# tenpy/cyten

Measured on AMD Instinct MI355X. Metric: block-sparse tdot+SVD GFLOP/s (fp64), higher is better.
Workload: dtype f64

## Files before the change

### cyten_amd/csrc/blocked_qr.hip

```cpp
#include "blocked_qr.h"
#include "qr_strip_chunks.h"

#include <algorithm>
#include <cstdlib>
#include <utility>

namespace cyb {
namespace {

#define GLOBAL_AS __attribute__((address_space(1)))
typedef GLOBAL_AS double* gp;
typedef const GLOBAL_AS double* gcp;
typedef double d4 __attribute__((ext_vector_type(4)));

constexpr int PNT = 512;
constexpr int PNW = PNT / 64;

__device__ __forceinline__ double wave_sum(double v)
{
#pragma unroll
    for (int o = 32; o > 0; o >>= 1) v += __shfl_xor(v, o);
    return v;
}

// ... 81 lines not shown
            else if (i > col) val = (tj != 0.0) ? x[i - col] * scale : 0.0;
            v[i] = val;
        }
        __syncthreads();
        if (tj != 0.0) {
            for (int c = col + 1 + wave; c < j0 + pw; c += PNW) {
                gp a = Ac + (int64_t)c * ld + col;
                gcp vv = v + col;
                double dot = 0.0;
                for (int i = lane; i < L; i += 64) dot += vv[i] * a[i];
                dot = wave_sum(dot) * tj;
                for (int i = lane; i < L; i += 64) a[i] -= dot * vv[i];
            }
        }
        for (int i = wave; i < jj; i += PNW) {
            gcp vi = V + (int64_t)(j0 + i) * ld;
            double dot = 0.0;
            for (int r = col + lane; r < m; r += 64) dot += vi[r] * v[r];
            dot = wave_sum(dot);
            if (lane == 0) z[i] = dot;
        }
        __syncthreads();
        if (tid < jj) {
            double acc = 0.0;
            for (int l = tid; l < jj; ++l) acc += Ts[tid][l] * z[l];
            Ts[tid][jj] = -tj * acc;
        }
        if (tid == 0) Ts[jj][jj] = tj;
        __syncthreads();
    }
    for (int e = tid; e < NBK * NBK; e += PNT) ((gp)d.T)[e] = Ts[e / NBK][e % NBK];
}

#ifndef CYB_QR_READLANE
#define CYB_QR_READLANE 1
#endif
constexpr int RP_NT = 512;
constexpr int RP_RPT = 3;
constexpr int RP_NW = RP_NT / 64;

__device__ __forceinline__ double dshfl_xor(double v, int m) { return __shfl_xor(v, m); }

#ifndef CYB_QR_REDUCE_DPP
#define CYB_QR_REDUCE_DPP 1
#endif
#if CYB_QR_REDUCE_DPP
__device__ __forceinline__ void dswap32(double& a, double& b)
{
    const auto lo = __builtin_amdgcn_permlane32_swap((unsigned)__double2loint(a), (unsigned)__double2loint(b), false, false);
    const auto hi = __builtin_amdgcn_permlane32_swap((unsigned)__double2hiint(a), (unsigned)__double2hiint(b), false, false);
    a = __hiloint2double((int)hi[0], (int)lo[0]);
    b = __hiloint2double((int)hi[1], (int)lo[1]);
}
__device__ __forceinline__ void dswap16(double& a, double& b)
{
    const auto lo = __builtin_amdgcn_permlane16_swap((unsigned)__double2loint(a), (unsigned)__double2loint(b), false, false);
    const auto hi = __builtin_amdgcn_permlane16_swap((unsigned)__double2hiint(a), (unsigned)__double2hiint(b), false, false);
    a = __hiloint2double((int)hi[0], (int)lo[0]);
    b = __hiloint2double((int)hi[1], (int)lo[1]);
}
template <int CTRL, int BANKS>
__device__ __forceinline__ double ddpp(double old, double src)
{
    const int lo = __builtin_amdgcn_update_dpp(__double2loint(old), __double2loint(src), CTRL, 0xf, BANKS, false);
    const int hi = __builtin_amdgcn_update_dpp(__double2hiint(old), __double2hiint(src), CTRL, 0xf, BANKS, false);
    return __hiloint2double(hi, lo);
}
__device__ __forceinline__ double reduce_scatter16(double (&v)[16], int )
{
    double a[8];
#pragma unroll
    for (int i = 0; i < 8; ++i) {
        double x = v[i], y = v[i + 8];
        dswap32(x, y);
        a[i] = x + y;
    }
    double b[4];
#pragma unroll
    for (int i = 0; i < 4; ++i) {
        double x = a[i], y = a[i + 4];
        dswap16(x, y);
        b[i] = x + y;
    }
    constexpr int ROW_MIRROR = 0x140, ROW_HALF_MIRROR = 0x141;
    double c[2];
#pragma unroll
    for (int i = 0; i < 2; ++i) {
        const double p = ddpp<ROW_MIRROR, 0xc>(b[i], b[i + 2]);
        const double q = ddpp<ROW_MIRROR, 0x3>(b[i + 2], b[i]);
        c[i] = p + q;
    }
    const double p = ddpp<ROW_HALF_MIRROR, 0xa>(c[0], c[1]);
    const double q = ddpp<ROW_HALF_MIRROR, 0x5>(c[1], c[0]);
    double d = p + q;
    d += ddpp<0x4e, 0xf>(d, d);
    d += ddpp<0xb1, 0xf>(d, d);
    return d;
}
#else
__device__ __forceinline__ double reduce_scatter16(double (&v)[16], int lane)
{
    double a[8];
    {
        const bool hi = (lane & 32) != 0;
#pragma unroll
        for (int i = 0; i < 8; ++i) {
            const double send = hi ? v[i] : v[i + 8];
            const double keep = hi ? v[i + 8] : v[i];
            a[i] = keep + dshfl_xor(send, 32);
        }
    }
    double b[4];
    {
        const bool hi = (lane & 16) != 0;
#pragma unroll
        for (int i = 0; i < 4; ++i) {
            const double send = hi ? a[i] : a[i + 4];
            const double keep = hi ? a[i + 4] : a[i];
            b[i] = keep + dshfl_xor(send, 16);
        }
    }
    double c[2];
    {
        const bool hi = (lane & 8) != 0;
#pragma unroll
        for (int i = 0; i < 2; ++i) {
            const double send = hi ? b[i] : b[i + 2];
            const double keep = hi ? b[i + 2] : b[i];
            c[i] = keep + dshfl_xor(send, 8);
        }
    }
    double d;
    {
        const bool hi = (lane & 4) != 0;
        const double send = hi ? c[0] : c[1];
        const double keep = hi ? c[1] : c[0];
        d = keep + dshfl_xor(send, 4);
    }
    d += dshfl_xor(d, 2);
    d += dshfl_xor(d, 1);
    return d;
}
#endif

struct PanelShared {
    double wred[2][RP_NW][NBK];
    double wsum[2][NBK];
    double rowb[2][NBK];
    double Zs[NBK][NBK + 1];
    double taus[NBK];
    double Ts[NBK][NBK + 1];
};

template <int JJ, int RPT, int NT>
__device__ __forceinline__ void panel_step(double (&P)[RPT][NBK], PanelShared& sh, const PanelDesc& d, int tid)
{
    if (JJ >= d.pw) return;
    const int lane = tid & 63, wave = tid >> 6;
    const int j0 = d.j0;
    const int prow = j0 + JJ;
    constexpr int pb = JJ & 1;
#pragma unroll
    for (int h = 0; h < 2; ++h) {
        double part[16];
#pragma unroll
        for (int c = 0; c < 16; ++c) part[c] = 0.0;
#pragma unroll
        for (int q = 0; q < RPT; ++q) {
            const double x = (q == 0 && tid <= JJ) ? 0.0 : P[q][JJ];
#pragma unroll
            for (int c = 0; c < 16; ++c) part[c] += x * P[q][h * 16 + c];
        }
        const double r = reduce_scatter16(part, lane);
        if ((lane & 3) == 0) {
            const int idx = ((lane >> 5) & 1) * 8 + ((lane >> 4) & 1) * 4 + ((lane >> 3) & 1) * 2 + ((lane >> 2) & 1);
            sh.wred[pb][wave][h * 16 + idx] = r;
        }
    }
    if (tid == JJ) {
#pragma unroll
        for (int c = 0; c < NBK; ++c) sh.rowb[pb][c] = P[0][c];
    }
    __syncthreads();
#if CYB_QR_READLANE
    const int lc = lane & (NBK - 1);
    double ws = 0.0;
#pragma unroll
    for (int w = 0; w < NT / 64; ++w) ws += sh.wred[pb][w][lc];
    const double rb = sh.rowb[pb][lc];
    const double alpha = __hiloint2double(__builtin_amdgcn_readlane(__double2hiint(rb), JJ), __builtin_amdgcn_readlane(__double2loint(rb), JJ));
    const double xn2_raw = __hiloint2double(__builtin_amdgcn_readlane(__double2hiint(ws), JJ), __builtin_amdgcn_readlane(__double2loint(ws), JJ));
#else
    if (tid < NBK) {
        double t = 0.0;
#pragma unroll
        for (int w = 0; w < NT / 64; ++w) t += sh.wred[pb][w][tid];
        sh.wsum[pb][tid] = t;
    }
    __syncthreads();
    const double alpha = sh.rowb[pb][JJ];
    const double xn2_raw = sh.wsum[pb][JJ];
#endif
    const double xn2 = fma(alpha * alpha, (d.pad & PANEL_REFLECT_ALWAYS) ? 1e-40 : 0.0, xn2_raw);
    double tau = 0.0, scale = 0.0, beta = alpha;
    if (xn2 > 1e-290) {
        beta = -copysign(sqrt(alpha * alpha + xn2), alpha);
        tau = (beta - alpha) / beta;
        scale = 1.0 / (alpha - beta);
    }
    double v[RPT];
#pragma unroll
    for (int q = 0; q < RPT; ++q) {
        const double x = P[q][JJ];
        if (q == 0) {
            const bool below = tid > JJ;
            const bool pivot = tid == JJ;
            v[q] = below ? x * scale : (pivot ? 1.0 : 0.0);
            P[q][JJ] = below ? v[q] : (pivot ? beta : x);
        } else {
            v[q] = x * scale;
            P[q][JJ] = v[q];
        }
    }
#if CYB_QR_READLANE
    const double tl = tau * (rb + scale * ws);
    const int tlo = __double2loint(tl), thi = __double2hiint(tl);
#pragma unroll
    for (int c = JJ + 1; c < NBK; ++c) {
        const double t = __hiloint2double(__builtin_amdgcn_readlane(thi, c), __builtin_amdgcn_readlane(tlo, c));
#pragma unroll
        for (int q = 0; q < RPT; ++q) P[q][c] -= t * v[q];
    }
#else
#pragma unroll
    for (int c = JJ + 1; c < NBK; ++c) {
        if (c < d.pw) {
            const double t = tau * (sh.rowb[pb][c] + scale * sh.wsum[pb][c]);
#pragma unroll
            for (int q = 0; q < RPT; ++q) P[q][c] -= t * v[q];
        }
    }
#endif
#if CYB_QR_READLANE
    if (tid < JJ) sh.Zs[tid][JJ] = rb + scale * ws;
#else
    if (tid < JJ) sh.Zs[tid][JJ] = sh.rowb[pb][tid] + scale * sh.wsum[pb][tid];
#endif
    if (tid == 0) {
        sh.taus[JJ] = tau;
        ((gp)d.tau)[prow] = tau;
    }
}

template <int RPT, int NT, int... Is>
__device__ __forceinline__ void panel_steps(double (&P)[RPT][NBK], PanelShared& sh, const PanelDesc& d, int tid,
                                            std::integer_sequence<int, Is...>)
{
    (panel_step<Is, RPT, NT>(P, sh, d, tid), ...);
}

template <int RPT, int NT = RP_NT>
__device__ __forceinline__ void panel_reg_body(const PanelDesc& d, PanelShared& sh, const int tid)
{
    gp Ac = (gp)d.Ac;
    gp V = (gp)d.V;
    const int64_t ld = d.ld;
    const int m = d.m, j0 = d.j0, pw = d.pw;
    double P[RPT][NBK];
#pragma unroll
    for (int q = 0; q < RPT; ++q) {
        const int row = j0 + tid + NT * q;
        const bool ok = row < m;
        gcp src = (gcp)Ac + (int64_t)j0 * ld + (ok ? row : j0);
#pragma unroll
        for (int c = 0; c < NBK; ++c) P[q][c] = src[(int64_t)(c < pw ? c : pw - 1) * ld];
#pragma unroll
        for (int c = 0; c < NBK; ++c) {
            asm volatile("" : "+v"(P[q][c]));
            P[q][c] = (ok && c < pw) ? P[q][c] : 0.0;
        }
    }
    for (int e = tid; e < NBK * (NBK + 1); e += NT) (&sh.Zs[0][0])[e] = 0.0;
    __syncthreads();

    panel_steps<RPT, NT>(P, sh, d, tid, std::make_integer_sequence<int, NBK>{});
#pragma unroll
    for (int q = 0; q < RPT; ++q) {
        const int row = j0 + tid + NT * q;
        if (row < m) {
            gp pa = Ac + (int64_t)j0 * ld + row;
            gp pv = V + (int64_t)j0 * ld + row;
#pragma unroll
            for (int c = 0; c < NBK; ++c)
                if (c < pw) {
                    pa[(int64_t)c * ld] = P[q][c];
                    pv[(int64_t)c * ld] = (q > 0 || tid > c) ? P[q][c] : (tid == c ? 1.0 : 0.0);
                }
        }
    }
    for (int64_t e = tid; e < ((d.pad & PANEL_V_ZEROED) ? 0 : (int64_t)j0 * pw); e += NT) {
        const int c = (int)(e / j0), row = (int)(e % j0);
        V[(int64_t)(j0 + c) * ld + row] = 0.0;
    }
    __syncthreads();
    if (tid < NBK) {
        double trow[NBK];
#pragma unroll
        for (int j = 0; j < NBK; ++j) {
            double acc = 0.0;
#pragma unroll
            for (int l = 0; l < j; ++l) acc += trow[l] * sh.Zs[l][j];
            const double tj = j < pw ? sh.taus[j] : 0.0;
            trow[j] = (tid < j) ? -tj * acc : (tid == j ? tj : 0.0);
            sh.Ts[tid][j] = trow[j];
        }
    }
    __syncthreads();

    for (int e = tid; e < NBK * NBK; e += NT) ((gp)d.T)[e] = sh.Ts[e / NBK][e % NBK];
}

template <int NT, typename Desc>
__device__ __forceinline__ bool panel_stop_check(const Desc& d, double* red, int tid, bool writer = true)
{
    if (!d.ctl) return false;
    gp ctl = (gp)d.ctl;
    const double stopped = ctl[0];
    if (stopped != 0.0) return (double)d.step >= stopped - 1.0;
    if (d.n_parts <= 0) return false;
    gcp parts = (gcp)d.parts;
    double t = 0.0;
    for (int i = tid; i < d.n_parts; i += NT) t += parts[i];
#pragma unroll
    for (int o = 32; o > 0; o >>= 1) t += __shfl_xor(t, o);
    if ((tid & 63) == 0) red[tid >> 6] = t;
    __syncthreads();
    double sum = 0.0;
#pragma unroll
    for (int w = 0; w < NT / 64; ++w) sum += red[w];
    const double ref = fmax(ctl[1], sum);
    const bool stop = sum <= d.rel2 * ref;
    __syncthreads();
    if (tid == 0 && writer) {
        if (stop) ctl[0] = (double)d.step + 1.0;
        else ctl[1] = ref;
    }
    return stop;
}

__global__ void __launch_bounds__(RP_NT) qr_panel_reg_kernel(const PanelDesc* __restrict__ descs)
{
    __shared__ PanelShared sh;
    const PanelDesc d = descs[blockIdx.x];
    if (panel_stop_check<RP_NT>(d, &sh.wsum[0][0], (int)threadIdx.x)) return;
    panel_reg_body<RP_RPT>(d, sh, (int)threadIdx.x);
}
struct PanelDescM {
    double* Ac;
    double* V;
    double* T;
    double* tau;
    double* xchg;
    unsigned int* ticket;
    unsigned int* err;
    int64_t ld;
    int32_t m, j0, pw, vzero;
    int32_t wg, n_wg, pad0, pad1;
    double* ctl = nullptr;
    const double* parts = nullptr;
    double rel2 = 0.0;
    int32_t n_parts = 0, step = 0;
};
constexpr int RPM_ROWS = RP_NT * RP_RPT;

template <int JJ>
__device__ __forceinline__ void panel_step_multi(double (&P)[RP_RPT][NBK], PanelShared& sh, const PanelDescM& d, int tid)
{
    if (JJ >= d.pw) return;
    const int lane = tid & 63, wave = tid >> 6;
    const int j0 = d.j0, rbase = d.j0 + d.wg * RPM_ROWS;
    const int prow = j0 + JJ;
    constexpr int pb = JJ & 1;
#pragma unroll
    for (int h = 0; h < 2; ++h) {
        double part[16];
#pragma unroll
        for (int c = 0; c < 16; ++c) part[c] = 0.0;
#pragma unroll
        for (int q = 0; q < RP_RPT; ++q) {
            const int row = rbase + tid + RP_NT * q;
            const double x = (row <= prow) ? 0.0 : P[q][JJ];
#pragma unroll
            for (int c = 0; c < 16; ++c) part[c] += x * P[q][h * 16 + c];
        }
        const double r = reduce_scatter16(part, lane);
        if ((lane & 3) == 0) {
            const int idx = ((lane >> 5) & 1) * 8 + ((lane >> 4) & 1) * 4 + ((lane >> 3) & 1) * 2 + ((lane >> 2) & 1);
            sh.wred[pb][wave][h * 16 + idx] = r;
        }
    }
#pragma unroll
    for (int q = 0; q < RP_RPT; ++q)
        if (rbase + tid + RP_NT * q == prow) {
#pragma unroll
            for (int c = 0; c < NBK; ++c) sh.rowb[pb][c] = P[q][c];
        }
    __syncthreads();
    if (tid < NBK) {
        double t = 0.0;
#pragma unroll
        for (int w = 0; w < RP_NW; ++w) t += sh.wred[pb][w][tid];
        double* slot = d.xchg + ((size_t)JJ * d.n_wg + d.wg) * 64;
        __hip_atomic_store(slot + tid, t, __ATOMIC_RELAXED, __HIP_MEMORY_SCOPE_AGENT);
        if (d.wg == 0) __hip_atomic_store(slot + 32 + tid, sh.rowb[pb][tid], __ATOMIC_RELAXED, __HIP_MEMORY_SCOPE_AGENT);
        asm volatile("s_waitcnt vmcnt(0)" ::: "memory");
        if (tid == 0) {
            __hip_atomic_fetch_add(d.ticket + JJ, 1u, __ATOMIC_RELAXED, __HIP_MEMORY_SCOPE_AGENT);
            const unsigned long long t0 = wall_clock64();
            while (__hip_atomic_load(d.ticket + JJ, __ATOMIC_RELAXED, __HIP_MEMORY_SCOPE_AGENT) < (unsigned int)d.n_wg) {
                if (wall_clock64() - t0 > 100000000ull || __hip_atomic_load(d.err, __ATOMIC_RELAXED, __HIP_MEMORY_SCOPE_AGENT)) {
                    __hip_atomic_store(d.err, 1u, __ATOMIC_RELAXED, __HIP_MEMORY_SCOPE_AGENT);
                    break;
                }
            }
        }
        asm volatile("" ::: "memory");
        __builtin_amdgcn_wave_barrier();
        double tot = 0.0;
        for (int w = 0; w < d.n_wg; ++w)
            tot += __hip_atomic_load(d.xchg + ((size_t)JJ * d.n_wg + w) * 64 + tid, __ATOMIC_RELAXED, __HIP_MEMORY_SCOPE_AGENT);
        sh.wsum[pb][tid] = tot;
        sh.rowb[pb][tid] = __hip_atomic_load(d.xchg + (size_t)JJ * d.n_wg * 64 + 32 + tid, __ATOMIC_RELAXED, __HIP_MEMORY_SCOPE_AGENT);
    }
    __syncthreads();
    const double alpha = sh.rowb[pb][JJ];
    const double xn2 = fma(alpha * alpha, (d.vzero & PANEL_REFLECT_ALWAYS) ? 1e-40 : 0.0, sh.wsum[pb][JJ]);
    double tau = 0.0, scale = 0.0, beta = alpha;
    if (xn2 > 1e-290) {
        beta = -copysign(sqrt(alpha * alpha + xn2), alpha);
        tau = (beta - alpha) / beta;
        scale = 1.0 / (alpha - beta);
    }
    double v[RP_RPT];
#pragma unroll
    for (int q = 0; q < RP_RPT; ++q) {
        const int row = rbase + tid + RP_NT * q;
        const double x = P[q][JJ];
        const bool below = row > prow;
        const bool pivot = row == prow;
        v[q] = below ? x * scale : (pivot ? 1.0 : 0.0);
        P[q][JJ] = below ? v[q] : (pivot ? beta : x);
    }
#pragma unroll
    for (int c = JJ + 1; c < NBK; ++c) {
        if (c < d.pw) {
            const double t = tau * (sh.rowb[pb][c] + scale * sh.wsum[pb][c]);
#pragma unroll
            for (int q = 0; q < RP_RPT; ++q) P[q][c] -= t * v[q];
        }
    }
    if (tid < JJ) sh.Zs[tid][JJ] = sh.rowb[pb][tid] + scale * sh.wsum[pb][tid];
    if (tid == 0) {
        sh.taus[JJ] = tau;
        if (d.wg == 0) ((gp)d.tau)[prow] = tau;
    }
}

template <int... Is>
__device__ __forceinline__ void panel_steps_multi(double (&P)[RP_RPT][NBK], PanelShared& sh, const PanelDescM& d, int tid,
                                                  std::integer_sequence<int, Is...>)
{
    (panel_step_multi<Is>(P, sh, d, tid), ...);
}

__global__ void __launch_bounds__(RP_NT) qr_panel_multi_kernel(const PanelDescM* __restrict__ descs)
{
    __shared__ PanelShared sh;
    const PanelDescM d = descs[blockIdx.x];
    const int tid = threadIdx.x;
    if (panel_stop_check<RP_NT>(d, &sh.wsum[0][0], tid, d.wg == 0)) return;
    gp Ac = (gp)d.Ac;
    gp V = (gp)d.V;
    const int64_t ld = d.ld;
    const int m = d.m, j0 = d.j0, pw = d.pw, rbase = d.j0 + d.wg * RPM_ROWS;
    double P[RP_RPT][NBK];
#pragma unroll
    for (int q = 0; q < RP_RPT; ++q) {
        const int row = rbase + tid + RP_NT * q;
#pragma unroll
        for (int c = 0; c < NBK; ++c) P[q][c] = (row < m && c < pw) ? Ac[(int64_t)(j0 + c) * ld + row] : 0.0;
    }
    for (int e = tid; e < NBK * (NBK + 1); e += RP_NT) (&sh.Zs[0][0])[e] = 0.0;
    __syncthreads();
    panel_steps_multi(P, sh, d, tid, std::make_integer_sequence<int, NBK>{});
#pragma unroll
    for (int q = 0; q < RP_RPT; ++q) {
        const int row = rbase + tid + RP_NT * q;
        if (row < m) {
#pragma unroll
            for (int c = 0; c < NBK; ++c)
                if (c < pw) {
                    const int col = j0 + c;
                    Ac[(int64_t)col * ld + row] = P[q][c];
                    V[(int64_t)col * ld + row] = (row > col) ? P[q][c] : (row == col ? 1.0 : 0.0);
                }
        }
    }
    if (d.wg == 0 && !(d.vzero & PANEL_V_ZEROED))
        for (int64_t e = tid; e < (int64_t)j0 * pw; e += RP_NT) {
            const int c = (int)(e / j0), row = (int)(e % j0);
            V[(int64_t)(j0 + c) * ld + row] = 0.0;
        }
    __syncthreads();
    if (tid < NBK) {
        double trow[NBK];
#pragma unroll
        for (int j = 0; j < NBK; ++j) {
            double acc = 0.0;
#pragma unroll
            for (int l = 0; l < j; ++l) acc += trow[l] * sh.Zs[l][j];
            const double tj = j < pw ? sh.taus[j] : 0.0;
            trow[j] = (tid < j) ? -tj * acc : (tid == j ? tj : 0.0);
            sh.Ts[tid][j] = trow[j];
        }
    }
    __syncthreads();
    if (d.wg == 0)
        for (int e = tid; e < NBK * NBK; e += RP_NT) ((gp)d.T)[e] = sh.Ts[e / NBK][e % NBK];
}

constexpr int RP_WAVE_RPT = 3;
constexpr int RP_WAVE_ROWS = 64 * RP_WAVE_RPT;
__global__ void __launch_bounds__(64) qr_panel_wave_kernel(const PanelDesc* __restrict__ descs)
{
    __shared__ PanelShared sh;
    const PanelDesc d = descs[blockIdx.x];
    if (panel_stop_check<64>(d, &sh.wsum[0][0], (int)threadIdx.x)) return;
    panel_reg_body<RP_WAVE_RPT, 64>(d, sh, (int)threadIdx.x);
}
__global__ void __launch_bounds__(128) qr_panel_wave2_kernel(const PanelDesc* __restrict__ descs)
{
    __shared__ PanelShared sh;
    const PanelDesc d = descs[blockIdx.x];
    if (panel_stop_check<128>(d, &sh.wsum[0][0], (int)threadIdx.x)) return;
    panel_reg_body<RP_WAVE_RPT, 128>(d, sh, (int)threadIdx.x);
}
__global__ void __launch_bounds__(256) qr_panel_wave4_kernel(const PanelDesc* __restrict__ descs)
{
    __shared__ PanelShared sh;
    const PanelDesc d = descs[blockIdx.x];
    if (panel_stop_check<256>(d, &sh.wsum[0][0], (int)threadIdx.x)) return;
    panel_reg_body<RP_WAVE_RPT, 256>(d, sh, (int)threadIdx.x);
}

struct StripDesc {
    double* C;
    const double* V;
    const double* T;
    int64_t ldc, ldv;
    int32_t mr, nc, pw, transT;
    const double* ctl = nullptr;
    double* part_out = nullptr;
    int32_t step = 0, pad2 = 0;
};
constexpr int ST_NT = 512;
constexpr int ST_NW = ST_NT / 64;
constexpr int ST_LS = NBK + 1;
constexpr int ST_UN = 4;

template <bool NORM>
__global__ void __launch_bounds__(ST_NT) reflector_strip_kernel(const StripDesc* __restrict__ descs)
{
    __shared__ double part[ST_NW][NBK][ST_LS];
    __shared__ double W1s[NBK][ST_LS], W2s[NBK][ST_LS], Ps[NBK][ST_LS];
    const StripDesc d = descs[blockIdx.x];
    if (d.ctl) {
        const double stopped = *(gcp)d.ctl;
        if (stopped != 0.0 && (double)d.step >= stopped - 1.0) return;
    }
    const int tid = threadIdx.x, lane = tid & 63, wave = tid >> 6;
    const int x = lane & 15, kq = lane >> 4;
    gcp V = (gcp)d.V;
    gp C = (gp)d.C;
    gcp T = (gcp)d.T;
    const int mr = d.mr, nc = d.nc, pw = d.pw;
    const int64_t ldv = d.ldv, ldc = d.ldc;
    for (int e = tid; e < NBK * NBK; e += ST_NT) {
        const int a = e / NBK, b = e % NBK;
        Ps[a][b] = T[d.transT ? b * NBK + a : e];
    }
    {
        const int64_t vo0 = (int64_t)(x < pw ? x : 0) * ldv, vo1 = (int64_t)(x + 16 < pw ? x + 16 : 0) * ldv;
        const int64_t co0 = (int64_t)(x < nc ? x : 0) * ldc, co1 = (int64_t)(x + 16 < nc ? x + 16 : 0) * ldc;
        d4 acc[2][2];
#pragma unroll
        for (int i = 0; i < 2; ++i)
#pragma unroll
            for (int j = 0; j < 2; ++j) acc[i][j] = d4{0.0, 0.0, 0.0, 0.0};
        const int nstep = (mr + 7) / 8;
        double va[ST_UN][2][2], ca[ST_UN][2][2], vn[ST_UN][2][2], cn[ST_UN][2][2];
        auto load = [&](double (&v)[ST_UN][2][2], double (&c)[ST_UN][2][2], int s0) {
#pragma unroll
            for (int u = 0; u < ST_UN; ++u) {
                const int i = (s0 + ST_NW * u) * 8 + 2 * kq;
#pragma unroll
                for (int h = 0; h < 2; ++h) {
                    const bool ok = i + h < mr;
                    const int ii = ok ? i + h : 0;
                    v[u][0][h] = ok ? V[vo0 + ii] : 0.0;
                    v[u][1][h] = ok ? V[vo1 + ii] : 0.0;
                    c[u][0][h] = ok ? C[co0 + ii] : 0.0;
                    c[u][1][h] = ok ? C[co1 + ii] : 0.0;
                }
            }
        };
        if (wave < nstep) load(va, ca, wave);
        for (int s0 = wave; s0 < nstep; s0 += ST_NW * ST_UN) {
            const bool more = s0 + ST_NW * ST_UN < nstep;
            if (more) load(vn, cn, s0 + ST_NW * ST_UN);
#pragma unroll
            for (int u = 0; u < ST_UN; ++u) {
                if (s0 + ST_NW * u < nstep) {
#pragma unroll
                    for (int h = 0; h < 2; ++h)
#pragma unroll
                        for (int i = 0; i < 2; ++i)
#pragma unroll
                            for (int j = 0; j < 2; ++j)
                                acc[i][j] = __builtin_amdgcn_mfma_f64_16x16x4f64(va[u][i][h], ca[u][j][h], acc[i][j], 0, 0, 0);
                }
            }
            if (more) {
#pragma unroll
                for (int u = 0; u < ST_UN; ++u)
#pragma unroll
                    for (int i = 0; i < 2; ++i)
#pragma unroll
                        for (int h = 0; h < 2; ++h) {
                            va[u][i][h] = vn[u][i][h];
                            ca[u][i][h] = cn[u][i][h];
                        }
            }
        }
#pragma unroll
        for (int i = 0; i < 2; ++i)
#pragma unroll
            for (int j = 0; j < 2; ++j)
#pragma unroll
                for (int r = 0; r < 4; ++r) part[wave][i * 16 + kq + 4 * r][j * 16 + x] = acc[i][j][r];
    }
    __syncthreads();
    for (int e = tid; e < NBK * NBK; e += ST_NT) {
        const int a = e / NBK, c = e % NBK;
        double t = 0.0;
#pragma unroll
        for (int w = 0; w < ST_NW; ++w) t += part[w][a][c];
        W1s[a][c] = t;
    }
    __syncthreads();
    if (wave < 4) {
        const int ta = wave >> 1, tc = wave & 1;
        d4 acc = d4{0.0, 0.0, 0.0, 0.0};
#pragma unroll
        for (int kk = 0; kk < NBK / 4; ++kk)
            acc = __builtin_amdgcn_mfma_f64_16x16x4f64(Ps[ta * 16 + x][4 * kk + kq], W1s[4 * kk + kq][tc * 16 + x], acc, 0, 0, 0);
#pragma unroll
        for (int r = 0; r < 4; ++r) W2s[ta * 16 + kq + 4 * r][tc * 16 + x] = acc[r];
    }
    __syncthreads();
    {
        double w2[2][NBK / 4];
#pragma unroll
        for (int ct = 0; ct < 2; ++ct)
#pragma unroll
            for (int kk = 0; kk < NBK / 4; ++kk) w2[ct][kk] = -W2s[4 * kk + kq][ct * 16 + x];
        int64_t vcol[NBK / 4], ccol[2][4];
#pragma unroll
        for (int kk = 0; kk < NBK / 4; ++kk) vcol[kk] = (int64_t)(4 * kk + kq < pw ? 4 * kk + kq : 0) * ldv;
#pragma unroll
        for (int ct = 0; ct < 2; ++ct)
#pragma unroll
            for (int r = 0; r < 4; ++r) {
                const int c = ct * 16 + kq + 4 * r;
                ccol[ct][r] = (int64_t)(c < nc ? c : 0) * ldc;
            }
        const int ntile = (mr + 15) / 16;
        struct Tile {
            double v[NBK / 4];
            d4 c[2];
        };
        auto load = [&](Tile& t, int rt) {
            const int i = rt * 16 + x;
            const bool ok = i < mr;
            const int ii = ok ? i : 0;
#pragma unroll
            for (int kk = 0; kk < NBK / 4; ++kk) t.v[kk] = ok ? V[vcol[kk] + ii] : 0.0;
#pragma unroll
            for (int ct = 0; ct < 2; ++ct)
#pragma unroll
                for (int r = 0; r < 4; ++r) t.c[ct][r] = C[ccol[ct][r] + ii];
        };
        double nrm2 = 0.0;
        auto finish = [&](Tile& t, int rt) {
#pragma unroll
            for (int kk = 0; kk < NBK / 4; ++kk) {
// ... 543 lines not shown
}
static size_t scratch_doubles(int64_t m, int64_t n, int64_t kc)
{
    const size_t strips = (size_t)(1 + kWSplit) * NBK * (size_t)std::max<int64_t>(std::max(n, kc), 1);
    const size_t wide = (size_t)w_split(m) * (size_t)wide_width() * (size_t)std::max<int64_t>(kc, 1);
    return std::max(strips, wide);
}

size_t bqr_aux_bytes(int64_t m, int64_t n, int64_t ld, int64_t kc)
{
    const int64_t k = std::min(m, n);
    const int64_t npan = (k + NBK - 1) / NBK;
    return al256(sizeof(double) * (size_t)ld * (size_t)std::max<int64_t>(k, 1)) + al256(sizeof(double) * (size_t)npan * NBK * NBK) +
           al256(sizeof(double) * (size_t)std::max<int64_t>(k, 1)) + al256(sizeof(double) * scratch_doubles(m, n, kc));
}

size_t bqr_carve(BqrMat& q, char* base, int64_t kc)
{
    const int64_t k = q.k;
    const int64_t npan = (k + NBK - 1) / NBK;
    size_t off = 0;
    q.V = reinterpret_cast<double*>(base + off);
    off += al256(sizeof(double) * (size_t)q.ld * (size_t)std::max<int64_t>(k, 1));
    q.T = reinterpret_cast<double*>(base + off);
    off += al256(sizeof(double) * (size_t)npan * NBK * NBK);
    q.tau = reinterpret_cast<double*>(base + off);
    off += al256(sizeof(double) * (size_t)std::max<int64_t>(k, 1));
    q.scratch = reinterpret_cast<double*>(base + off);
    q.scr_half = (int64_t)NBK * std::max<int64_t>(std::max<int64_t>(q.n, kc), 1);
    q.scr_total = (int64_t)scratch_doubles(q.m, q.n, kc);
    off += al256(sizeof(double) * (size_t)q.scr_total);
    return off;
}

template <typename Desc>
static void set_panel_stop(Desc& d, const BqrMat& q, int n_parts, int step)
{
    d.ctl = q.ctl;
    d.parts = q.parts;
    d.rel2 = q.stop_rel2;
    d.n_parts = n_parts;
    d.step = step;
}

int bqr_factor(cyb_ctx_t ctx, const std::vector<BqrMat>& mats)
{
    auto pflags = [](const BqrMat& q) { return (q.v_zeroed ? PANEL_V_ZEROED : 0) | (q.reflect_always ? PANEL_REFLECT_ALWAYS : 0); };
    int max_pan = 0;
    for (const auto& q : mats) max_pan = std::max(max_pan, (q.k + NBK - 1) / NBK);
    struct Step {
        size_t off_pd = 0, off_pdr = 0, off_pdm = 0;
        unsigned n_pd = 0, n_pdr = 0, n_pdm = 0;
        int wave = 0;
        StripStep strips;
    };
    std::vector<Step> steps;
    std::vector<char> image;
    static const bool no_multi = getenv("CYB_QR_NOMULTI") != nullptr;
    static const bool no_reg = getenv("CYB_QR_PANEL_GLOBAL") != nullptr;
    static const bool no_wave = getenv("CYB_QR_NOWAVE") != nullptr;
    std::vector<size_t> x_off(mats.size(), 0);
    size_t x_bytes = 0, n_multi_wg = 0;
    const size_t t_bytes = al256(sizeof(unsigned int) * NBK * mats.size());
    for (size_t qi = 0; qi < mats.size(); ++qi) {
        const int wmax = (mats[qi].m + RPM_ROWS - 1) / RPM_ROWS;
        if (mats[qi].m > RPM_ROWS && std::min(mats[qi].m, mats[qi].n) > 0) {
            x_off[qi] = t_bytes + 256 + x_bytes;
            x_bytes += sizeof(double) * NBK * (size_t)wmax * 64;
            n_multi_wg += (size_t)wmax;
        }
    }
    const bool multi = !no_multi && x_bytes > 0 && n_multi_wg <= (size_t)ctx->n_cu;
    char* xbase = nullptr;
    if (multi) {
        void* xw = nullptr;
        CYB_TRY(ctx->workspace(al256(t_bytes + 256 + x_bytes), &xw, 3));
        xbase = static_cast<char*>(xw);
        CYB_HIP(hipMemsetAsync(xbase + t_bytes, 0, 256, ctx->stream));
    }
    static const bool no_stop = getenv("CYB_QR_NOSTOP") != nullptr;
    auto stoppable = [&](const BqrMat& q) {
        return !no_stop && !no_reg && q.ctl && q.parts && q.stop_rel2 > 0.0 && (q.m <= RPM_ROWS || multi);
    };
    size_t n_slots = 0;
    for (const auto& q : mats) n_slots += (size_t)((q.n + NBK - 1) / NBK) * (size_t)bqr_strip_slots(q.m);
    double* wsplit = nullptr;
    CYB_TRY(split_workspace(ctx, n_slots, &wsplit));
    std::vector<int> n_parts_prev(mats.size(), 0);
    static const int stop_every = std::max(1, getenv("CYB_QR_STOP_EVERY") ? atoi(getenv("CYB_QR_STOP_EVERY")) : 2);
    for (StepChunks c(max_pan); c.more(); c.next()) {
        steps.clear();
        image.clear();
        for (int p = c.begin; p < c.end; ++p) {
            std::vector<PanelDesc> pd, pd_reg;
            std::vector<PanelDescM> pdm;
            std::vector<StripDesc> sd;
            std::vector<std::pair<int, int>> cnt;
            for (const auto& q : mats) {
                const int j0 = p * NBK;
                if (j0 >= q.k) continue;
                const int64_t nt = q.n - (j0 + std::min(NBK, q.k - j0));
                if (nt > 0) cnt.push_back({q.m - j0, (int)((nt + NBK - 1) / NBK)});
            }
            const int step_ch = step_chunk_rows(cnt, ctx->n_cu);
            Step st;
            for (size_t qi = 0; qi < mats.size(); ++qi) {
                const auto& q = mats[qi];
                const int j0 = p * NBK;
                if (j0 >= q.k) continue;
                const int pw = std::min(NBK, q.k - j0);
                double* Tp = q.T + (size_t)p * NBK * NBK;
                const bool stop = stoppable(q);
                if (!no_reg && q.m - j0 <= RPM_ROWS) {
                    pd_reg.push_back(PanelDesc{q.Ac, q.V, Tp, q.tau, q.ld, q.m, j0, pw, pflags(q)});
                    if (stop) set_panel_stop(pd_reg.back(), q, n_parts_prev[qi], p);
                } else if (multi && !no_reg) {
                    const int n_wg = (q.m - j0 + RPM_ROWS - 1) / RPM_ROWS;
                    for (int w = 0; w < n_wg; ++w) {
                        pdm.push_back(PanelDescM{q.Ac, q.V, Tp, q.tau, reinterpret_cast<double*>(xbase + x_off[qi]),
                                                 reinterpret_cast<unsigned int*>(xbase) + qi * NBK, reinterpret_cast<unsigned int*>(xbase + t_bytes),
                                                 q.ld, q.m, j0, pw, pflags(q), w, n_wg, 0, 0});
                        if (stop) set_panel_stop(pdm.back(), q, n_parts_prev[qi], p);
                    }
                } else
                    pd.push_back(PanelDesc{q.Ac, q.V, Tp, q.tau, q.ld, q.m, j0, pw, pflags(q) & PANEL_REFLECT_ALWAYS});
                const int j1 = j0 + pw;
                const int64_t nt = q.n - j1, mr = q.m - j0;
                n_parts_prev[qi] = 0;
                if (nt <= 0) continue;
                const size_t s_begin = sd.size();
                add_strips(sd, q.Ac + (size_t)j1 * q.ld + j0, q.ld, nt, q.V + (size_t)j0 * q.ld + j0, q.ld, Tp, mr, pw, 1);
                if (stop) {
                    const bool measure = p % stop_every == stop_every - 1;
                    const int nch = strip_chunks((int)mr, step_ch);
                    for (size_t si = s_begin; si < sd.size(); ++si) {
                        sd[si].ctl = q.ctl;
                        sd[si].part_out = measure ? q.parts + (si - s_begin) * (size_t)nch : nullptr;
                        sd[si].step = p;
                    }
                    if (measure) {
                        n_parts_prev[qi] = (int)(sd.size() - s_begin) * nch;
                        st.strips.norm = true;
                    }
                }
            }
            st.n_pd = (unsigned)pd.size();
            st.n_pdr = (unsigned)pd_reg.size();
            st.n_pdm = (unsigned)pdm.size();
            if (st.n_pd) st.off_pd = put(image, pd.data(), sizeof(PanelDesc) * pd.size());
            if (st.n_pdr) st.off_pdr = put(image, pd_reg.data(), sizeof(PanelDesc) * pd_reg.size());
            if (st.n_pdm) st.off_pdm = put(image, pdm.data(), sizeof(PanelDescM) * pdm.size());
            int max_rows = 0;
            for (const auto& d : pd_reg) max_rows = std::max(max_rows, d.m - d.j0);
            st.wave = (no_wave || st.n_pdr == 0) ? 0 : max_rows <= RP_WAVE_ROWS ? 1 : max_rows <= 2 * RP_WAVE_ROWS ? 2 : max_rows <= 4 * RP_WAVE_ROWS ? 4 : 0;
            st.strips.stage(sd, step_ch, wsplit, image);
            steps.push_back(st);
        }
        void* d_image = nullptr;
        CYB_TRY(ctx->upload(image.data(), image.size(), &d_image));
        char* dbase = static_cast<char*>(d_image);
        for (const Step& st : steps) {
            if (st.n_pd)
                hipLaunchKernelGGL(qr_panel_kernel, dim3(st.n_pd), dim3(PNT), 0, ctx->stream,
                                   reinterpret_cast<const PanelDesc*>(dbase + st.off_pd));
            if (st.n_pdm) {
                CYB_HIP(hipMemsetAsync(xbase, 0, t_bytes, ctx->stream));
                hipLaunchKernelGGL(qr_panel_multi_kernel, dim3(st.n_pdm), dim3(RP_NT), 0, ctx->stream,
                                   reinterpret_cast<const PanelDescM*>(dbase + st.off_pdm));
            }
            if (st.n_pdr && st.wave == 1)
                hipLaunchKernelGGL(qr_panel_wave_kernel, dim3(st.n_pdr), dim3(64), 0, ctx->stream,
                                   reinterpret_cast<const PanelDesc*>(dbase + st.off_pdr));
            else if (st.n_pdr && st.wave == 2)
                hipLaunchKernelGGL(qr_panel_wave2_kernel, dim3(st.n_pdr), dim3(128), 0, ctx->stream,
                                   reinterpret_cast<const PanelDesc*>(dbase + st.off_pdr));
            else if (st.n_pdr && st.wave == 4)
                hipLaunchKernelGGL(qr_panel_wave4_kernel, dim3(st.n_pdr), dim3(256), 0, ctx->stream,
                                   reinterpret_cast<const PanelDesc*>(dbase + st.off_pdr));
            else if (st.n_pdr)
                hipLaunchKernelGGL(qr_panel_reg_kernel, dim3(st.n_pdr), dim3(RP_NT), 0, ctx->stream,
                                   reinterpret_cast<const PanelDesc*>(dbase + st.off_pdr));
            CYB_HIP(hipGetLastError());
            CYB_TRY(st.strips.launch(ctx, d_image));
        }
    }
    if (multi) {
        unsigned int h_err = 0;
        CYB_HIP(hipMemcpyAsync(&h_err, xbase + t_bytes, sizeof(unsigned int), hipMemcpyDeviceToHost, ctx->stream));
        CYB_HIP(hipStreamSynchronize(ctx->stream));
        if (h_err) {
            set_error("blocked QR: a workgroup of the multi-workgroup panel kernel waited more than a second for its partners");
            return CYB_ERR_HIP;
        }
    }
    return CYB_OK;
}

static int apply_q_strips(cyb_ctx_t ctx, const std::vector<BqrMat>& mats, const std::vector<BqrTarget>& targets)
{
    int max_pan = 0;
    for (const auto& t : targets) max_pan = std::max(max_pan, (mats[(size_t)t.mat].k + NBK - 1) / NBK);
    size_t n_slots = 0;
    for (const auto& t : targets) n_slots += (size_t)((t.kc + NBK - 1) / NBK) * (size_t)bqr_strip_slots(mats[(size_t)t.mat].m);
    double* wsplit = nullptr;
    CYB_TRY(split_workspace(ctx, n_slots, &wsplit));
    std::vector<StripStep> steps;
    std::vector<char> image;
    for (StepChunks c(max_pan); c.more(); c.next()) {
        steps.clear();
        image.clear();
        for (int i = c.begin; i < c.end; ++i) {
            const int p = max_pan - 1 - i;
            std::vector<StripDesc> sd;
            for (const auto& t : targets) {
                const BqrMat& q = mats[(size_t)t.mat];
                const int j0 = p * NBK;
                if (j0 >= q.k || t.kc <= 0) continue;
                CYB_REQUIRE((int64_t)NBK * t.kc <= q.scr_half, "bqr_apply_q: target wider than the carved scratch");
                const size_t s_begin = sd.size();
                add_strips(sd, t.C + j0, t.ldc, t.kc, q.V + (size_t)j0 * q.ld + j0, q.ld, q.T + (size_t)p * NBK * NBK, q.m - j0, std::min(NBK, q.k - j0), 0);
                if (q.ctl && q.stop_rel2 > 0.0)
                    for (size_t si = s_begin; si < sd.size(); ++si) {
                        sd[si].ctl = q.ctl;
                        sd[si].step = p;
                    }
            }
            if (sd.empty()) continue;
            std::vector<std::pair<int, int>> cnt;
            for (const auto& d : sd) cnt.push_back({d.mr, 1});
            StripStep st;
            st.stage(sd, step_chunk_rows(cnt, ctx->n_cu), wsplit, image);
            steps.push_back(st);
        }
        if (steps.empty()) continue;
        void* d_image = nullptr;
        CYB_TRY(ctx->upload(image.data(), image.size(), &d_image));
        for (const auto& st : steps) CYB_TRY(st.launch(ctx, d_image));
    }
    return CYB_OK;
}

static int apply_q_wide(cyb_ctx_t ctx, const std::vector<BqrMat>& mats, const std::vector<BqrTarget>& targets)
{
    const int W = wide_width();
    struct Tgt {
        const BqrMat* q;
        const BqrTarget* t;
        int k_eff, ng;
        double* VT;
        double* TS;
        double* G;
        std::vector<int> n_gp;
    };
    std::vector<Tgt> tg;
    size_t bytes = 0;
    int max_ng = 0;
    for (const auto& t : targets) {
        const BqrMat& q = mats[(size_t)t.mat];
        const int npan = (q.k + NBK - 1) / NBK;
        const int nf = t.n_pan >= 0 ? std::min(npan, (int)t.n_pan) : npan;
        const int k_eff = std::min<int>(q.k, nf * NBK);
        if (k_eff <= 0 || t.kc <= 0) continue;
        Tgt g{&q, &t, k_eff, (k_eff + W - 1) / W, nullptr, nullptr, nullptr, {}};
        CYB_REQUIRE((int64_t)w_split(q.m) * W * t.kc <= q.scr_total, "bqr_apply_q: target wider than the carved scratch");
        for (int s = 0; s < g.ng; ++s) {
            const int j0 = s * W, w = std::min(W, k_eff - j0);
            const int min_rows = q.m - j0 - (w - 1) / NBK * NBK;
            g.n_gp.push_back(std::max(1, std::min(4, min_rows / 256)));
        }
        max_ng = std::max(max_ng, g.ng);
        tg.push_back(std::move(g));
    }
    if (tg.empty()) return CYB_OK;
    std::vector<size_t> o_vt(tg.size()), o_ts(tg.size()), o_g(tg.size());
    for (size_t i = 0; i < tg.size(); ++i) {
        size_t n_g = 0;
        for (int n : tg[i].n_gp) n_g += (size_t)n;
        o_vt[i] = bytes;
        bytes += al256(sizeof(double) * (size_t)tg[i].q->ld * (size_t)tg[i].k_eff);
        o_ts[i] = bytes;
        bytes += al256(sizeof(double) * (size_t)tg[i].ng * W * W);
        o_g[i] = bytes;
        bytes += al256(sizeof(double) * n_g * W * W);
    }
    void* ws = nullptr;
    CYB_TRY(ctx->workspace(bytes, &ws, 5));
    for (size_t i = 0; i < tg.size(); ++i) {
        tg[i].VT = reinterpret_cast<double*>(static_cast<char*>(ws) + o_vt[i]);
        tg[i].TS = reinterpret_cast<double*>(static_cast<char*>(ws) + o_ts[i]);
        tg[i].G = reinterpret_cast<double*>(static_cast<char*>(ws) + o_g[i]);
    }
    std::vector<char> image;
    {
        GemmBatch gg, gv;
        std::vector<MergeDesc> md;
        for (const Tgt& g : tg) {
            const BqrMat& q = *g.q;
            size_t gp0 = 0;
            for (int s = 0; s < g.ng; ++s) {
                const int j0 = s * W, w = std::min(W, g.k_eff - j0), n_gp = g.n_gp[(size_t)s];
                const double* Vs = q.V + (size_t)j0 * q.ld + j0;
                double* Gs = g.G + gp0 * (size_t)W * W;
                double* TSs = g.TS + (size_t)s * W * W;
                for (int a = NBK; a < w; a += NBK) {
                    const int wb = std::min(NBK, w - a);
                    const int64_t rows = q.m - j0 - a, chunk = (rows + n_gp - 1) / n_gp;
                    for (int p = 0; p < n_gp; ++p) {
                        const int64_t r0 = a + chunk * p, kr = std::min(chunk, rows - chunk * p);
                        gg.add(Gs + (size_t)p * W * W + a, a, wb, W, Vs + r0, q.ld, 1, Vs + (size_t)a * q.ld + r0, 1, q.ld, kr, 1.0, 0.0);
                    }
                }
                md.push_back(MergeDesc{Gs, q.T + (size_t)(j0 / NBK) * NBK * NBK, TSs, (int64_t)W * W, w, W, n_gp, 0});
                gv.add(g.VT + (size_t)j0 * q.ld + j0, w, q.m - j0, q.ld, TSs, 1, W, Vs, q.ld, 1, w, 1.0, 0.0);
                gp0 += (size_t)n_gp;
            }
        }
        GemmStaged sg, sv;
        CYB_TRY(gg.stage(ctx, image, sg));
        CYB_TRY(gv.stage(ctx, image, sv));
        const size_t off_md = (image.size() + 255) / 256 * 256;
        image.resize(off_md + sizeof(MergeDesc) * md.size());
        memcpy(image.data() + off_md, md.data(), sizeof(MergeDesc) * md.size());
        void* d_image = nullptr;
        CYB_TRY(ctx->upload(image.data(), image.size(), &d_image));
        CYB_TRY(gemm_launch_staged(ctx, sg, d_image));
        const MergeDesc* mdp = reinterpret_cast<const MergeDesc*>(static_cast<char*>(d_image) + off_md);
        if (W <= 128) hipLaunchKernelGGL(merge_t_kernel<96>, dim3((unsigned)md.size()), dim3(MG_NT), 0, ctx->stream, mdp);
        else hipLaunchKernelGGL(merge_t_kernel<224>, dim3((unsigned)md.size()), dim3(MG_NT), 0, ctx->stream, mdp);
        CYB_HIP(hipGetLastError());
        CYB_TRY(gemm_launch_staged(ctx, sv, d_image));
// ... 110 lines not shown
```

Measured before the change: 6161.

## Add two-half recursive tall-panel QR kernel with 16-column register tiles

Adds a 256-thread tall-panel QR kernel for register panels that exceed the wave-kernel row limits. It factors the 32-column panel as two 16-column halves, applying the first half's compact-WY update to the second half through shared-memory W products and readlane broadcasts. It then builds the T factor from cross-half Z terms. This halves the per-thread register tile compared with the full-width register kernel, aiming for better occupancy and less register pressure. In exchange it adds extra global passes over the trailing columns and more synchronisation.

```diff
diff --git a/cyten_amd/csrc/blocked_qr.hip b/cyten_amd/csrc/blocked_qr.hip
--- a/cyten_amd/csrc/blocked_qr.hip
+++ b/cyten_amd/csrc/blocked_qr.hip
@@ -257,22 +257,23 @@
     double Ts[NBK][NBK + 1];
 };
 
-template <int JJ, int RPT, int NT>
-__device__ __forceinline__ void panel_step(double (&P)[RPT][NBK], PanelShared& sh, const PanelDesc& d, int tid)
-{
-    if (JJ >= d.pw) return;
+template <int JJ, int RPT, int NT, int NB = NBK, int OFF = 0>
+__device__ __forceinline__ void panel_step(double (&P)[RPT][NB], PanelShared& sh, const PanelDesc& d, int tid)
+{
+    constexpr int GJ = OFF + JJ;
+    if (GJ >= d.pw) return;
     const int lane = tid & 63, wave = tid >> 6;
     const int j0 = d.j0;
-    const int prow = j0 + JJ;
+    const int prow = j0 + GJ;
     constexpr int pb = JJ & 1;
 #pragma unroll
-    for (int h = 0; h < 2; ++h) {
+    for (int h = 0; h < NB / 16; ++h) {
         double part[16];
 #pragma unroll
         for (int c = 0; c < 16; ++c) part[c] = 0.0;
 #pragma unroll
         for (int q = 0; q < RPT; ++q) {
-            const double x = (q == 0 && tid <= JJ) ? 0.0 : P[q][JJ];
+            const double x = (q == 0 && tid <= GJ) ? 0.0 : P[q][JJ];
 #pragma unroll
             for (int c = 0; c < 16; ++c) part[c] += x * P[q][h * 16 + c];
         }
@@ -282,13 +283,13 @@
             sh.wred[pb][wave][h * 16 + idx] = r;
         }
     }
-    if (tid == JJ) {
-#pragma unroll
-        for (int c = 0; c < NBK; ++c) sh.rowb[pb][c] = P[0][c];
+    if (tid == GJ) {
+#pragma unroll
+        for (int c = 0; c < NB; ++c) sh.rowb[pb][c] = P[0][c];
     }
     __syncthreads();
 #if CYB_QR_READLANE
-    const int lc = lane & (NBK - 1);
+    const int lc = lane & (NB - 1);
     double ws = 0.0;
 #pragma unroll
     for (int w = 0; w < NT / 64; ++w) ws += sh.wred[pb][w][lc];
@@ -296,7 +297,7 @@
     const double alpha = __hiloint2double(__builtin_amdgcn_readlane(__double2hiint(rb), JJ), __builtin_amdgcn_readlane(__double2loint(rb), JJ));
     const double xn2_raw = __hiloint2double(__builtin_amdgcn_readlane(__double2hiint(ws), JJ), __builtin_amdgcn_readlane(__double2loint(ws), JJ));
 #else
-    if (tid < NBK) {
+    if (tid < NB) {
         double t = 0.0;
 #pragma unroll
         for (int w = 0; w < NT / 64; ++w) t += sh.wred[pb][w][tid];
@@ -318,8 +319,8 @@
     for (int q = 0; q < RPT; ++q) {
         const double x = P[q][JJ];
         if (q == 0) {
-            const bool below = tid > JJ;
-            const bool pivot = tid == JJ;
+            const bool below = tid > GJ;
+            const bool pivot = tid == GJ;
             v[q] = below ? x * scale : (pivot ? 1.0 : 0.0);
             P[q][JJ] = below ? v[q] : (pivot ? beta : x);
         } else {
@@ -331,15 +332,15 @@
     const double tl = tau * (rb + scale * ws);
     const int tlo = __double2loint(tl), thi = __double2hiint(tl);
 #pragma unroll
-    for (int c = JJ + 1; c < NBK; ++c) {
+    for (int c = JJ + 1; c < NB; ++c) {
         const double t = __hiloint2double(__builtin_amdgcn_readlane(thi, c), __builtin_amdgcn_readlane(tlo, c));
 #pragma unroll
         for (int q = 0; q < RPT; ++q) P[q][c] -= t * v[q];
     }
 #else
 #pragma unroll
-    for (int c = JJ + 1; c < NBK; ++c) {
-        if (c < d.pw) {
+    for (int c = JJ + 1; c < NB; ++c) {
+        if (OFF + c < d.pw) {
             const double t = tau * (sh.rowb[pb][c] + scale * sh.wsum[pb][c]);
 #pragma unroll
             for (int q = 0; q < RPT; ++q) P[q][c] -= t * v[q];
@@ -347,21 +348,38 @@
     }
 #endif
 #if CYB_QR_READLANE
-    if (tid < JJ) sh.Zs[tid][JJ] = rb + scale * ws;
+    if (tid < JJ) sh.Zs[OFF + tid][GJ] = rb + scale * ws;
 #else
-    if (tid < JJ) sh.Zs[tid][JJ] = sh.rowb[pb][tid] + scale * sh.wsum[pb][tid];
+    if (tid < JJ) sh.Zs[OFF + tid][GJ] = sh.rowb[pb][tid] + scale * sh.wsum[pb][tid];
 #endif
     if (tid == 0) {
-        sh.taus[JJ] = tau;
+        sh.taus[GJ] = tau;
         ((gp)d.tau)[prow] = tau;
     }
 }
 
-template <int RPT, int NT, int... Is>
-__device__ __forceinline__ void panel_steps(double (&P)[RPT][NBK], PanelShared& sh, const PanelDesc& d, int tid,
+template <int RPT, int NT, int NB = NBK, int OFF = 0, int... Is>
+__device__ __forceinline__ void panel_steps(double (&P)[RPT][NB], PanelShared& sh, const PanelDesc& d, int tid,
                                             std::integer_sequence<int, Is...>)
 {
-    (panel_step<Is, RPT, NT>(P, sh, d, tid), ...);
+    (panel_step<Is, RPT, NT, NB, OFF>(P, sh, d, tid), ...);
+}
+
+template <int N>
+__device__ __forceinline__ void panel_t_rows(PanelShared& sh, int pw, int tid)
+{
+    if (tid < N) {
+        double trow[N];
+#pragma unroll
+        for (int j = 0; j < N; ++j) {
+            double acc = 0.0;
+#pragma unroll
+            for (int l = 0; l < j; ++l) acc += trow[l] * sh.Zs[l][j];
+            const double tj = j < pw ? sh.taus[j] : 0.0;
+            trow[j] = (tid < j) ? -tj * acc : (tid == j ? tj : 0.0);
+            sh.Ts[tid][j] = trow[j];
+        }
+    }
 }
 
 template <int RPT, int NT = RP_NT>
@@ -408,18 +426,7 @@
         V[(int64_t)(j0 + c) * ld + row] = 0.0;
     }
     __syncthreads();
-    if (tid < NBK) {
-        double trow[NBK];
-#pragma unroll
-        for (int j = 0; j < NBK; ++j) {
-            double acc = 0.0;
-#pragma unroll
-            for (int l = 0; l < j; ++l) acc += trow[l] * sh.Zs[l][j];
-            const double tj = j < pw ? sh.taus[j] : 0.0;
-            trow[j] = (tid < j) ? -tj * acc : (tid == j ? tj : 0.0);
-            sh.Ts[tid][j] = trow[j];
-        }
-    }
+    panel_t_rows<NBK>(sh, pw, tid);
     __syncthreads();
 
     for (int e = tid; e < NBK * NBK; e += NT) ((gp)d.T)[e] = sh.Ts[e / NBK][e % NBK];
@@ -656,6 +663,216 @@
     const PanelDesc d = descs[blockIdx.x];
     if (panel_stop_check<256>(d, &sh.wsum[0][0], (int)threadIdx.x)) return;
     panel_reg_body<RP_WAVE_RPT, 256>(d, sh, (int)threadIdx.x);
+}
+
+constexpr int TP_NT = 256;
+constexpr int TP_RPT = 6;
+constexpr int TP_NB = 16;
+constexpr int TP_NW = TP_NT / 64;
+static_assert(TP_NT * TP_RPT == RP_NT * RP_RPT && 2 * TP_NB == NBK && TP_NT == TP_NB * TP_NB, "tall panel kernel: shape");
+
+struct TallShared {
+    double Wp[TP_NW][TP_NB][TP_NB];
+    double Ws[TP_NB][TP_NB + 1];
+    double W2[TP_NB][TP_NB];
+};
+
+template <typename T>
+__device__ __forceinline__ GLOBAL_AS T* tall_at(GLOBAL_AS T* col, unsigned byte_off)
+{
+    typedef typename std::conditional<std::is_const<T>::value, const GLOBAL_AS char, GLOBAL_AS char>::type B;
+    asm volatile("" : "+v"(byte_off));
+    return (GLOBAL_AS T*)((B*)col + byte_off);
+}
+
+__device__ __forceinline__ void tall_rows(unsigned (&rsafe)[TP_RPT], const PanelDesc& d, int tid)
+{
+    asm volatile("" : "+v"(tid));
+#pragma unroll
+    for (int q = 0; q < TP_RPT; ++q) rsafe[q] = 8u * (unsigned)(d.j0 + tid + TP_NT * q < d.m ? tid + TP_NT * q : 0);
+}
+
+template <int OFF>
+__device__ __forceinline__ void tall_load(double (&P)[TP_RPT][TP_NB], const PanelDesc& d, const unsigned (&rsafe)[TP_RPT], int tid)
+{
+    gcp col = (gcp)d.Ac + (int64_t)(d.j0 + OFF) * d.ld + d.j0;
+#pragma unroll
+    for (int c = 0; c < TP_NB; ++c) {
+#pragma unroll
+        for (int q = 0; q < TP_RPT; ++q) P[q][c] = *tall_at(col, rsafe[q]);
+        if (OFF + c + 1 < d.pw) col += d.ld;
+    }
+#pragma unroll
+    for (int q = 0; q < TP_RPT; ++q) {
+        const bool ok = d.j0 + tid + TP_NT * q < d.m;
+#pragma unroll
+        for (int c = 0; c < TP_NB; ++c) {
+            asm volatile("" : "+v"(P[q][c]));
+            P[q][c] = (ok && OFF + c < d.pw) ? P[q][c] : 0.0;
+        }
+    }
+}
+
+template <int OFF>
+__device__ __forceinline__ void tall_put(const double (&P)[TP_RPT][TP_NB], gp X, const PanelDesc& d, const unsigned (&rsafe)[TP_RPT], int tid)
+{
+#pragma unroll
+    for (int q = 0; q < TP_RPT; ++q)
+        if (d.j0 + tid + TP_NT * q < d.m) {
+            gp col = X + (int64_t)(d.j0 + OFF) * d.ld + d.j0;
+#pragma unroll
+            for (int c = 0; c < TP_NB; ++c, col += d.ld)
+                if (OFF + c < d.pw) *tall_at(col, rsafe[q]) = P[q][c];
+        }
+}
+
+template <int OFF>
+__device__ __forceinline__ void tall_store(double (&P)[TP_RPT][TP_NB], const PanelDesc& d, const unsigned (&rsafe)[TP_RPT], int tid)
+{
+    tall_put<OFF>(P, (gp)d.Ac, d, rsafe, tid);
+#pragma unroll
+    for (int c = 0; c < TP_NB; ++c) {
+        asm volatile("" : "+v"(P[0][c]));
+        P[0][c] = (OFF + c < d.pw) ? (tid > OFF + c ? P[0][c] : (tid == OFF + c ? 1.0 : 0.0)) : 0.0;
+    }
+    tall_put<OFF>(P, (gp)d.V, d, rsafe, tid);
+}
+
+__device__ __forceinline__ void tall_column(double (&x)[TP_RPT], gcp col, const unsigned (&rsafe)[TP_RPT])
+{
+#pragma unroll
+    for (int q = 0; q < TP_RPT; ++q) x[q] = *tall_at(col, rsafe[q]);
+}
+
+__device__ __forceinline__ void tall_dots(const double (&P)[TP_RPT][TP_NB], double (&x)[TP_RPT], gcp next, int k,
+                                          const unsigned (&rsafe)[TP_RPT], TallShared& ts, int tid)
+{
+    const int lane = tid & 63, wave = tid >> 6;
+    double part[TP_NB];
+#pragma unroll
+    for (int c = 0; c < TP_NB; ++c) part[c] = 0.0;
+    double y[TP_RPT];
+#pragma unroll
+    for (int q = 0; q < TP_RPT; ++q) y[q] = x[q];
+    tall_column(x, next, rsafe);
+#pragma unroll
+    for (int q = 0; q < TP_RPT; ++q) {
+        asm volatile("" : "+v"(y[q]));
+#pragma unroll
+        for (int c = 0; c < TP_NB; ++c) part[c] += y[q] * P[q][c];
+    }
+    const double r = reduce_scatter16(part, lane);
+    if ((lane & 3) == 0) {
+        const int idx = ((lane >> 5) & 1) * 8 + ((lane >> 4) & 1) * 4 + ((lane >> 3) & 1) * 2 + ((lane >> 2) & 1);
+        ts.Wp[wave][k][idx] = r;
+    }
+}
+
+template <bool FULL>
+__device__ __forceinline__ void panel_tall_body(PanelDesc d, PanelShared& sh, TallShared& ts, const int tid)
+{
+    if (FULL) d.pw = NBK;
+    gp Ac = (gp)d.Ac;
+    gp V = (gp)d.V;
+    const int64_t ld = d.ld;
+    const int m = d.m, j0 = d.j0, pw = d.pw;
+    unsigned rsafe[TP_RPT];
+    tall_rows(rsafe, d, tid);
+    double P[TP_RPT][TP_NB];
+    tall_load<0>(P, d, rsafe, tid);
+    for (int e = tid; e < NBK * (NBK + 1); e += TP_NT) (&sh.Zs[0][0])[e] = 0.0;
+    __syncthreads();
+    panel_steps<TP_RPT, TP_NT, TP_NB, 0>(P, sh, d, tid, std::make_integer_sequence<int, TP_NB>{});
+    tall_rows(rsafe, d, tid);
+    tall_store<0>(P, d, rsafe, tid);
+    if (pw > TP_NB) {
+        __syncthreads();
+        const int nr = pw - TP_NB;
+        gp cp = Ac + (int64_t)(j0 + TP_NB) * ld + j0;
+        double x[TP_RPT];
+        tall_column(x, (gcp)cp, rsafe);
+#pragma unroll 1
+        for (int j = 0; j < nr; ++j) {
+            if (j + 1 < nr) cp += ld;
+            tall_dots(P, x, (gcp)cp, j, rsafe, ts, tid);
+        }
+        panel_t_rows<TP_NB>(sh, pw, tid);
+        __syncthreads();
+        const int tc = tid & (TP_NB - 1), tj = tid >> 4;
+        {
+            double s = 0.0;
+#pragma unroll
+            for (int w = 0; w < TP_NW; ++w) s += ts.Wp[w][tj][tc];
+            ts.Ws[tj][tc] = s;
+        }
+        __syncthreads();
+        {
+            double a = 0.0;
+#pragma unroll
+            for (int l = 0; l < TP_NB; ++l) a += sh.Ts[l][tc] * ts.Ws[tj][l];
+            ts.W2[tj][tc] = a;
+        }
+        __syncthreads();
+        cp = Ac + (int64_t)(j0 + TP_NB) * ld + j0;
+        tall_column(x, (gcp)cp, rsafe);
+#pragma unroll 1
+        for (int j = 0; j < nr; ++j) {
+            gp next = cp + (j + 1 < nr ? ld : 0);
+            const double w2 = ts.W2[j][tc];
+            const int wlo = __double2loint(w2), whi = __double2hiint(w2);
+            double y[TP_RPT];
+#pragma unroll
+            for (int q = 0; q < TP_RPT; ++q) y[q] = x[q];
+            tall_column(x, (gcp)next, rsafe);
+#pragma unroll
+            for (int c = 0; c < TP_NB; ++c) {
+                const double w = __hiloint2double(__builtin_amdgcn_readlane(whi, c), __builtin_amdgcn_readlane(wlo, c));
+#pragma unroll
+                for (int q = 0; q < TP_RPT; ++q) y[q] -= P[q][c] * w;
+            }
+#pragma unroll
+            for (int q = 0; q < TP_RPT; ++q)
+                if (j0 + tid + TP_NT * q < m) *tall_at(cp, rsafe[q]) = y[q];
+            cp = next;
+        }
+        tall_load<TP_NB>(P, d, rsafe, tid);
+        panel_steps<TP_RPT, TP_NT, TP_NB, TP_NB>(P, sh, d, tid, std::make_integer_sequence<int, TP_NB>{});
+        tall_rows(rsafe, d, tid);
+        tall_store<TP_NB>(P, d, rsafe, tid);
+        gcp vp = (gcp)V + (int64_t)j0 * ld + j0;
+        tall_column(x, vp, rsafe);
+#pragma unroll 1
+        for (int c = 0; c < TP_NB; ++c) {
+            if (c + 1 < TP_NB) vp += ld;
+            tall_dots(P, x, vp, c, rsafe, ts, tid);
+        }
+        __syncthreads();
+        {
+            double s = 0.0;
+#pragma unroll
+            for (int w = 0; w < TP_NW; ++w) s += ts.Wp[w][tj][tc];
+            sh.Zs[tj][TP_NB + tc] = s;
+        }
+    }
+    for (int64_t e = tid; e < ((d.pad & PANEL_V_ZEROED) ? 0 : (int64_t)j0 * pw); e += TP_NT) {
+        const int c = (int)(e / j0), row = (int)(e % j0);
+        V[(int64_t)(j0 + c) * ld + row] = 0.0;
+    }
+    __syncthreads();
+    panel_t_rows<NBK>(sh, pw, tid);
+    __syncthreads();
+    for (int e = tid; e < NBK * NBK; e += TP_NT) ((gp)d.T)[e] = sh.Ts[e / NBK][e % NBK];
+}
+
+__global__ void __launch_bounds__(TP_NT) qr_panel_tall_kernel(const PanelDesc* __restrict__ descs)
+{
+    __shared__ PanelShared sh;
+    __shared__ TallShared ts;
+    const PanelDesc d = descs[blockIdx.x];
+    const int tid = threadIdx.x;
+    if (panel_stop_check<TP_NT>(d, &sh.wsum[0][0], tid)) return;
+    if (d.pw == NBK) panel_tall_body<true>(d, sh, ts, tid);
+    else panel_tall_body<false>(d, sh, ts, tid);
 }
 
 struct StripDesc {
@@ -1505,7 +1722,7 @@
             if (st.n_pdm) st.off_pdm = put(image, pdm.data(), sizeof(PanelDescM) * pdm.size());
             int max_rows = 0;
             for (const auto& d : pd_reg) max_rows = std::max(max_rows, d.m - d.j0);
-            st.wave = (no_wave || st.n_pdr == 0) ? 0 : max_rows <= RP_WAVE_ROWS ? 1 : max_rows <= 2 * RP_WAVE_ROWS ? 2 : max_rows <= 4 * RP_WAVE_ROWS ? 4 : 0;
+            st.wave = (no_wave || st.n_pdr == 0) ? 0 : max_rows <= RP_WAVE_ROWS ? 1 : max_rows <= 2 * RP_WAVE_ROWS ? 2 : max_rows <= 4 * RP_WAVE_ROWS ? 4 : 6;
             st.strips.stage(sd, step_ch, wsplit, image);
             steps.push_back(st);
         }
@@ -1529,6 +1746,9 @@
                                    reinterpret_cast<const PanelDesc*>(dbase + st.off_pdr));
             else if (st.n_pdr && st.wave == 4)
                 hipLaunchKernelGGL(qr_panel_wave4_kernel, dim3(st.n_pdr), dim3(256), 0, ctx->stream,
+                                   reinterpret_cast<const PanelDesc*>(dbase + st.off_pdr));
+            else if (st.n_pdr && st.wave == 6)
+                hipLaunchKernelGGL(qr_panel_tall_kernel, dim3(st.n_pdr), dim3(TP_NT), 0, ctx->stream,
                                    reinterpret_cast<const PanelDesc*>(dbase + st.off_pdr));
             else if (st.n_pdr)
                 hipLaunchKernelGGL(qr_panel_reg_kernel, dim3(st.n_pdr), dim3(RP_NT), 0, ctx->stream,
```

Result: slower. 6069 (-1.5%).
